# jibo27/3DGS_Hierarchical_Training

Measured on AMD Instinct MI355X. Metric: train-step images/sec + fwd+bwd ms @1M Gaussians, 980x545; 1/2/4/8 GPU, higher is better.
Workload: dtype f32

## Files before the change

3dgs_hierarchical_training_amd/csrc/gsr_kernels.hip:

```cpp
#include <hip/hip_runtime.h>
#include <hip/hip_ext.h>
#include <type_traits>
#include <stdint.h>
#include <stdio.h>
#include <string.h>

#include <algorithm>
#include <atomic>
#include <chrono>
#include <cmath>
#include <map>
#include <mutex>
#include <tuple>
#include <vector>

#include "../../include/gsr.h"
#include "gsr_math.h"
#include "adam_math.h"
#include "radix_sort.h"
#include "blend_common.h"

#ifndef GSR_K9_UNROLL
#define GSR_K9_UNROLL 2
#endif
// ... 1877 lines not shown
    float C0 = 0.f, C1 = 0.f, C2 = 0.f, Dd = 0.f, Aa = 0.f;
    uint32_t last = 0;
    float g0 = 0.f, g1 = 0.f, g2 = 0.f;
    uint32_t lastp = 0u, id_rec = 0u;
    bool uni = false;
    if constexpr (IMP) {
        if (inside) {
            const size_t Pl = (size_t)W * H, P = Pl * (size_t)(T / Tl), pl = (size_t)py * W + px, pid = (size_t)bimg * Pl + pl;
            const float* oc = imp.color + (size_t)bimg * 3 * Pl + pl;
            const float o0 = oc[0], o1 = oc[Pl], o2 = oc[2 * Pl];
            g0 = (o0 >= 0.f && o0 <= 1.f) ? 1.f : 0.f;
            g1 = (o1 >= 0.f && o1 <= 1.f) ? 1.f : 0.f;
            g2 = (o2 >= 0.f && o2 <= 1.f) ? 1.f : 0.f;
            lastp = reinterpret_cast<const uint32_t*>(img)[P + pid];
        }
        const bool want = lastp > 0u && (g0 + g1 + g2) > 0.f;
        if (!__any(want)) return;
        Tr = want ? 1.f : -1.f;
        if (!want) g0 = g1 = g2 = 0.f;
        uni = __all(g0 == g1 && g1 == g2);
        imp.s_sum[0][lane] = 0.f; imp.s_sum[1][lane] = 0.f; imp.s_sum[2][lane] = 0.f;
    }
    float4 ra = {0, 0, 0, 0}, rb = ra, rc = ra;
    constexpr float kL2E = 1.4426950408889634f;
    const float sbx0 = (float)(tx * kTile + (sub & 1) * 8) - 0.5f * (float)W, sby0 = (float)(ty * kTile + (sub >> 1) * 8) - 0.5f * (float)H;
    const float sbx1 = fminf(sbx0 + 7.f, (float)(W - 1) - 0.5f * (float)W), sby1 = fminf(sby0 + 7.f, (float)(H - 1) - 0.5f * (float)H);
    uint32_t id_nn = 0u;
    auto fetch = [&](uint32_t id) {
        const float4* sp = reinterpret_cast<const float4*>(splat + id);
        ra = sp[0]; rb = sp[1]; rc = sp[2];
    };
    if (n > 0) {
        id_rec = list[rg.x + min(lane, n - 1)];
        fetch(id_rec);
        id_nn = list[rg.x + min(NT + lane, n - 1)];
    }
    int batches = 0;
    for (int b = 0; b < nb; b++) {
        const int buf = b & (kFwdBufs - 1);
        if (__all(Tr < 0.f)) break;
        if constexpr (!LEAN) {
        if (ckpt && !(b & 1) && (b >> 1) >= kCkptFirst) {
            float* c = ckpt + ((size_t)(rg.x >> 7) + tile + (b >> 1) - kCkptFirst) * kCkptFloats + sub * 64 + lane;
            c[0] = fabsf(Tr); c[256] = C0; c[512] = C1; c[768] = C2; c[1024] = Dd; c[1280] = Aa;
        }
        }
#ifdef GSR_K6_TIMING
        dbg_mark = __builtin_readcyclecounter();
#endif
        const int cnt = min(NT, n - b * NT);
        const bool reach_me = box_accept(make_tile_test(ra.x, ra.y, ra.z, ra.w, rb.x, rb.y), sbx0, sby0, sbx1, sby1);
        {
            const uint32_t lo = __float_as_uint(rc.w);
            ra.x = pixel_rel(ra.x, pixel_lo_x(lo), tox); ra.y = pixel_rel(ra.y, pixel_lo_y(lo), toy);
        }
        ra.z *= -0.5f * kL2E; ra.w *= -kL2E; rb.x *= -0.5f * kL2E;
        s_ab[buf][lane] = ra; s_ab[kFwdBufs + buf][lane] = rb;
        if constexpr (IMP) imp.s_id[lane] = id_rec;
        else s_c[buf][lane] = make_float2(rc.x, rc.y);
        const unsigned long long reach = __ballot(reach_me && lane < cnt);
        visits += (uint32_t)__popcll(reach);
        __builtin_amdgcn_fence(__ATOMIC_RELEASE, "wavefront");
        __builtin_amdgcn_wave_barrier();
        __builtin_amdgcn_fence(__ATOMIC_ACQUIRE, "wavefront");
        batches = b + 1;
#ifdef GSR_K6_TIMING
        { const unsigned long long t = __builtin_readcyclecounter(); dbg_stage += t - dbg_mark; dbg_mark = t; }
#endif
        const int nxt = (b + 1) * NT + lane;
        fetch(id_nn);
        if constexpr (IMP) id_rec = id_nn;
        id_nn = list[rg.x + min(nxt + NT, n - 1)];
        auto alpha_of = [&](int j, float& p2) {
            const float4 A = s_ab[buf][j];
            const float2 Bq = *reinterpret_cast<const float2*>(&s_ab[kFwdBufs + buf][j]);
            const float dx = A.x - pxf, dy = A.y - pyf;
            p2 = fmaf(Bq.x * dy, dy, fmaf(A.w, dy, A.z * dx) * dx);
#if defined(__HIP_DEVICE_COMPILE__)
            return fminf(kAlphaMax, Bq.y * __builtin_amdgcn_exp2f(p2));
#else
            return fminf(kAlphaMax, Bq.y * exp2f(p2));
#endif
        };
        auto blend = [&](int j, float p2, float alpha) {
            const bool inl = !IMP || (uint32_t)(b * NT + j + 1) <= lastp;
            const bool hit = !(p2 > 0.f) && !(alpha < kAlphaMin) && inl;
#ifdef GSR_K6_TIMING
            dbg_visits++;
#endif
            if constexpr (IMP) {
                if ((__builtin_amdgcn_ballot_w64(!(p2 > 0.f)) & __builtin_amdgcn_ballot_w64(!(alpha < kAlphaMin)) & __builtin_amdgcn_ballot_w64(inl)) == 0ull) return;
            } else {
                if ((__builtin_amdgcn_ballot_w64(!(p2 > 0.f)) & __builtin_amdgcn_ballot_w64(!(alpha < kAlphaMin))) == 0ull) return;
            }
#ifdef GSR_K6_TIMING
            dbg_taken++;
#endif
            const float4 B = s_ab[kFwdBufs + buf][j];
            float2 C = {0.f, 0.f};
            if constexpr (!IMP) C = s_c[buf][j];
            const float am = hit ? alpha : 0.f;
            const float test_T = Tr * (1.f - am);
            const bool pass = !(test_T < kTStop);
            const float asel = pass ? am : 0.f;
            const float w = asel * Tr;
            C0 = fmaf(B.w, w, C0); C1 = fmaf(C.x, w, C1); C2 = fmaf(C.y, w, C2);
            if constexpr (HAS_DA) { Dd = fmaf(B.z, w, Dd); Aa = fmaf(Tr, asel, Aa); }
            Tr = pass ? test_T : -fabsf(Tr);
            last = (pass && hit) ? (uint32_t)(b * NT + j + 1) : last;
            if constexpr (IMP) {
                if (uni) {
                    const float t = wave_reduce_one(w * g0);
                    if (lane == 0) atomicAdd(&imp.s_sum[0][j], t);
                } else {
                    const float t = wave_reduce_three(w * g0, w * g1, w * g2, lane);
                    if (lane < 12 && !(lane & 3)) atomicAdd(&imp.s_sum[lane >> 2][j], t);
                }
            }
        };
        for (unsigned long long rm = reach; rm != 0ull;) {
            const int j = (int)__builtin_ctzll(rm);
#if defined(__HIP_DEVICE_COMPILE__)
            asm("s_bitset0_b64 %0, %1" : "+s"(rm) : "s"(j));
#else
            rm &= rm - 1ull;
#endif
            float p2;
            const float a1 = alpha_of(j, p2);
            blend(j, p2, a1);
        }
#ifdef GSR_K6_TIMING
        dbg_loop += __builtin_readcyclecounter() - dbg_mark;
#endif
        if constexpr (IMP) {
            __builtin_amdgcn_fence(__ATOMIC_RELEASE, "wavefront");
            __builtin_amdgcn_wave_barrier();
            __builtin_amdgcn_fence(__ATOMIC_ACQUIRE, "wavefront");
            const int c = lane & 3;
#pragma unroll
            for (int q = 0; q < 4; q++) {
                const int jj = q * 16 + (lane >> 2);
                if (c < 3 && jj < cnt) {
                    const float v = imp.s_sum[uni ? 0 : c][jj];
                    if (v != 0.f) atomicAdd(imp.S + (size_t)imp.s_id[jj] * kImpStride + c, v);
                }
            }
            __builtin_amdgcn_fence(__ATOMIC_RELEASE, "wavefront");
            __builtin_amdgcn_wave_barrier();
            __builtin_amdgcn_fence(__ATOMIC_ACQUIRE, "wavefront");
            imp.s_sum[0][lane] = 0.f; imp.s_sum[1][lane] = 0.f; imp.s_sum[2][lane] = 0.f;
        }
    }
    if constexpr (IMP) return;
    if constexpr (!LEAN) { if (lane == 0) staged4[tile * 4 + sub] = (uint32_t)min(n, batches * NT); }
    if (cost_out && lane == 0) cost_out[xcd + 8 * kslot] = (uint16_t)min(visits, 65535u);
    if (cut_pass) {
        const bool live = !__all(Tr < 0.f);
        if (lane == 0) {
            if (cut_pass == 1 && live && cut.tend[tile] < cut.tbase[tile + 1]) {
                if (atomicExch(&cut.flag[tile], 1u) == 0u) atomicAdd(&cut.ctl[2], 1u);
            } else {
                uint32_t k = live ? kCutOpenKey : 0u;
                if (!live && batches > 0) {
                    const int lb = batches - 1, lc = min(NT, n - lb * NT);
                    k = __float_as_uint(s_ab[kFwdBufs + (lb & (kFwdBufs - 1))][lc - 1].z);
                }
                const uint32_t e = cut.cur[0] < (uint32_t)kVcEntries ? cut.cur[0] : 0u;
                if (k) atomicMax(cut.key + (size_t)e * (size_t)T + tile, k);
            }
        }
    }
#ifdef GSR_K6_TIMING
    if (lane == 0 && xcd + 8 * kslot < 65536) {
        unsigned long long* d = g_k6_dbg + 4 * (size_t)(xcd + 8 * kslot);
        d[0] = dbg_t0; d[1] = wall_clock64();
        d[2] = ((unsigned long long)__builtin_amdgcn_s_getreg((31 << 11) | 20) << 32) | (unsigned long long)__builtin_amdgcn_s_getreg((31 << 11) | 4);
        d[3] = ((unsigned long long)(uint32_t)n << 32) | (uint32_t)(batches * NT);
        g_k6_cnt[2 * (size_t)(xcd + 8 * kslot)] = dbg_visits; g_k6_cnt[2 * (size_t)(xcd + 8 * kslot) + 1] = dbg_taken;
        g_k6_cyc[2 * (size_t)(xcd + 8 * kslot)] = dbg_stage; g_k6_cyc[2 * (size_t)(xcd + 8 * kslot) + 1] = dbg_loop;
    }
#endif
    if (inside) {
        const size_t Pl = (size_t)W * H, P = Pl * (size_t)(T / Tl), pl = (size_t)py * W + px, pid = (size_t)bimg * Pl + pl;
        const float Tf = fabsf(Tr);
        if constexpr (!LEAN) {
            img[pid] = Tf;
            reinterpret_cast<uint32_t*>(img)[P + pid] = last;
            img[2 * P + pid] = C0; img[3 * P + pid] = C1; img[4 * P + pid] = C2;
            img[5 * P + pid] = Dd; img[6 * P + pid] = Aa;
        }
        float* oc = out_color + (size_t)bimg * 3 * Pl + pl;
        const float o0 = C0 + Tf * bg[0], o1 = C1 + Tf * bg[1], o2 = C2 + Tf * bg[2];
        oc[0] = o0;
        oc[Pl] = o1;
        oc[2 * Pl] = o2;
        if (out_clamped) {
            float* cc = out_clamped + (size_t)bimg * 3 * Pl + pl;
            cc[0] = o0 < 0.f ? 0.f : (o0 > 1.f ? 1.f : o0);
            cc[Pl] = o1 < 0.f ? 0.f : (o1 > 1.f ? 1.f : o1);
            cc[2 * Pl] = o2 < 0.f ? 0.f : (o2 > 1.f ? 1.f : o2);
        }
        if constexpr (HAS_DA) {
            out_depth[pid] = Dd;
            out_alpha[pid] = Aa;
        }
    }
}


__device__ __forceinline__ void blend_fwd_slot(const BlendBalance& bb, const bool table, int& kslot, uint16_t*& cost_out)
{
    if (bb.hdr) {
// ... 1548 lines not shown

#ifdef GSR_K8_PHASES
int gsr_debug_k8_phases(unsigned long long* host_dst) { return (int)hipMemcpyFromSymbol(host_dst, HIP_SYMBOL(g_k8ph), sizeof(unsigned long long) * 8 * 8192); }
#endif
#ifdef GSR_OS_TIMING
int gsr_debug_os_timing(unsigned long long* host_dst) { return (int)hipMemcpyFromSymbol(host_dst, HIP_SYMBOL(g_os_dbg), sizeof(unsigned long long) * 8 * 4096); }
int gsr_debug_gh_timing(unsigned long long* host_dst) { return (int)hipMemcpyFromSymbol(host_dst, HIP_SYMBOL(g_gh_dbg), sizeof(unsigned long long) * 8 * 512); }
#endif
#ifdef GSR_K9_TIMING
int gsr_debug_k9_timing(unsigned long long* host_dst, int reset)
{
    (void)reset;
    return (int)hipMemcpyFromSymbol(host_dst, HIP_SYMBOL(g_k9_dbg), sizeof(unsigned long long) * 8 * kK9DbgWaves);
}
#endif
#ifdef GSR_DB_TIMING
int gsr_debug_db_timing(unsigned long long* host_dst) { return (int)hipMemcpyFromSymbol(host_dst, HIP_SYMBOL(g_db_dbg), sizeof(unsigned long long) * 16); }
#endif
#ifdef GSR_K6_TIMING
int gsr_debug_k6_timing(unsigned long long* host_dst, int blocks)
{
    return (int)hipMemcpyFromSymbol(host_dst, HIP_SYMBOL(g_k6_dbg), sizeof(unsigned long long) * 4 * (size_t)blocks);
}
int gsr_debug_k6_counts(uint32_t* host_dst, int blocks)
{
    return (int)hipMemcpyFromSymbol(host_dst, HIP_SYMBOL(g_k6_cnt), sizeof(uint32_t) * 2 * (size_t)blocks);
}
int gsr_debug_k6_cycles(unsigned long long* host_dst, int blocks)
{
    return (int)hipMemcpyFromSymbol(host_dst, HIP_SYMBOL(g_k6_cyc), sizeof(unsigned long long) * 2 * (size_t)blocks);
}
int gsr_debug_k8_timing(unsigned long long* host_dst, int blocks)
{
    return (int)hipMemcpyFromSymbol(host_dst, HIP_SYMBOL(g_k8_dbg), sizeof(unsigned long long) * 4 * (size_t)blocks);
}
#endif
int gsr_set_option(const char* name, int value)
{
    if (!name) return GSR_ERR_ARG;
    if (!strcmp(name, "blend_fwd_ppt")) return (value == 0 || value == 7) ? GSR_OK : GSR_ERR_ARG;
    if (!strcmp(name, "ab_variants")) return 0;
    if (!strcmp(name, "bwd_split")) { if (value < 0 || value > 64) return GSR_ERR_ARG; g_bwd_split = value; return GSR_OK; }
    if (!strcmp(name, "ckpt_first")) { if (value < 1 || value > 64) return GSR_ERR_ARG; g_ckpt_first = value; return GSR_OK; }
    if (!strcmp(name, "tile_map")) return value == 2 ? GSR_OK : GSR_ERR_ARG;
    if (!strcmp(name, "blend_balance")) { g_blend_balance = value ? 1 : 0; return GSR_OK; }
    if (!strcmp(name, "early_r")) { g_early_r = value ? 1 : 0; return GSR_OK; }
    if (!strcmp(name, "list_cut")) { g_list_cut = value < 0 || value > 2 ? 1 : value; return GSR_OK; }
    if (!strcmp(name, "list_cut_min_n")) { g_list_cut_min_n = value < 0 ? 2000000 : value; return GSR_OK; }
    if (!strcmp(name, "view_cache_reset")) {
        int dev_id = 0;
        if (hipGetDevice(&dev_id) != hipSuccess || hipDeviceSynchronize() != hipSuccess) return GSR_ERR_HIP;
        std::lock_guard<std::mutex> lk(g_state_mutex);
        for (auto& c : g_view_costs)
            if (c.dev == dev_id && hipMemset(c.mem, 0, c.bytes) != hipSuccess) return GSR_ERR_HIP;
        return GSR_OK;
    }
    if (!strcmp(name, "list_cut_margin_e3")) { g_list_cut_margin_e3 = value < 0 ? 50 : value; return GSR_OK; }
    if (!strcmp(name, "list_cut_deep")) { g_list_cut_deep = value < 0 ? 8 : value; return GSR_OK; }
    if (!strcmp(name, "debug_late_bias")) { g_debug_late_bias = value; return GSR_OK; }
    if (!strcmp(name, "tile_sort")) { if (value < 0 || value > 2) return GSR_ERR_ARG; g_tile_sort = value; return GSR_OK; }
    if (!strcmp(name, "tile_sort_max_avg")) { if (value < 0) return GSR_ERR_ARG; g_tile_sort_max_avg = value; return GSR_OK; }
    if (!strcmp(name, "view_pose_tol_e6")) { if (value < 0) return GSR_ERR_ARG; g_view_pose_tol_e6 = value; return GSR_OK; }
    if (!strcmp(name, "depth_sort9")) { g_depth_sort9 = value ? 1 : 0; return GSR_OK; }
    if (!strcmp(name, "direct_binning")) { g_direct_bin = value ? 1 : 0; return GSR_OK; }
    if (!strcmp(name, "speculative_binning")) { g_speculate = value ? 1 : 0; return GSR_OK; }
    if (!strcmp(name, "deterministic_backward")) { g_deterministic = value ? 1 : 0; return GSR_OK; }
    if (!strcmp(name, "binning_capacity_hint")) {
        std::lock_guard<std::mutex> lk(g_state_mutex);
        g_hint_override = value > 0 ? value : -1;
        return GSR_OK;
    }
    if (!strcmp(name, "reset_speculation")) {
        std::lock_guard<std::mutex> lk(g_state_mutex);
        g_hints.clear(); g_hint_override = -1;
        g_spec_overflows = 0; g_spec_forwards = 0; g_exact_forwards = 0; g_depth_window_resorts = 0;
        g_full_depth_sort.clear();
        return GSR_OK;
    }
    if (!strcmp(name, "profile")) { g_profile = (value == 2 || value == 3) ? value : (value ? 1 : 0); g_profile_tick = 0; return GSR_OK; }
    if (!strcmp(name, "prep_hist_max_n")) { g_prep_hist_max_n = value; return GSR_OK; }
    if (!strcmp(name, "small_sort9")) { if (value < 0) return GSR_ERR_ARG; g_small_sort9 = value; return GSR_OK; }
    if (!strcmp(name, "poll_iters")) { g_poll_iters = value < 0 ? 0 : value; return GSR_OK; }
    if (!strcmp(name, "emit_hist")) { g_emit_hist = value ? 1 : 0; return GSR_OK; }
    if (!strcmp(name, "sort_algo")) return value == 2 ? GSR_OK : GSR_ERR_ARG;
    if (!strcmp(name, "blend_bwd_ppt")) return (value == 0 || value == 2) ? GSR_OK : GSR_ERR_ARG;
    return GSR_ERR_ARG;
}

struct DirectBinScratch { size_t M, GT, tbase, bsum, cut_chunk, cut_tend, cut_flag, cut_ctl, cut_bkey, cut_hist, bytes; };
static bool direct_bin_geometry(int N, int T, DirectBin& db, DirectBinScratch& ds)
{
    if (N < 1 || T < 1 || T > kDbMaxTiles) return false;
    static std::atomic<int> cus_cached{0};
    int cus = cus_cached.load(std::memory_order_relaxed);
    if (!cus) {
        int dev = 0, n = 0;
        cus = (hipGetDevice(&dev) == hipSuccess && hipDeviceGetAttribute(&n, hipDeviceAttributeMultiprocessorCount, dev) == hipSuccess && n > 0) ? n : 256;
        cus_cached.store(cus, std::memory_order_relaxed);
    }
    db.N = N; db.T = T; db.Tp = (T + 63) & ~63;
    const int lds = 12 * db.Tp + 4 * kDbPairs;
    const int per_cu = std::min(16, (160 * 1024) / lds);
    const long long resident = std::max<long long>(1, (long long)cus * per_cu);
    const int min_s = 128;
    long long S = ((long long)N + resident - 1) / resident;
    S = std::max<long long>(min_s, (S + 63) & ~63ll);
    if (S > 65472) return false;
    db.S = (int)S;
    db.NC = (int)(((long long)N + S - 1) / S);
    int G = 1;
    while (G * G < db.NC) G++;
    db.Cg = std::max(1, std::min((db.NC + G - 1) / G, 65535 / db.S));
    db.G = (db.NC + db.Cg - 1) / db.Cg;
    if (db.G > kDbMaxGroups) return false;
    size_t o = 0;
    ds.M = o; o += align256((size_t)db.NC * db.Tp * sizeof(uint16_t));
    ds.GT = o; o += align256((size_t)db.G * db.Tp * sizeof(uint32_t));
    ds.tbase = o; o += align256((size_t)(db.Tp + 1) * sizeof(uint32_t));
    ds.bsum = o; o += align256((size_t)db.G * ((db.Tp + 255) / 256) * sizeof(uint32_t));
    ds.cut_chunk = o; o += align256((size_t)db.Tp * sizeof(uint16_t));
    ds.cut_tend = o; o += align256((size_t)db.Tp * sizeof(uint32_t));
    ds.cut_flag = o; o += align256((size_t)db.Tp * sizeof(uint32_t));
    ds.cut_ctl = o; o += 256;
    ds.cut_bkey = o; o += align256((size_t)db.NC * sizeof(uint32_t));
    ds.cut_hist = o; o += align256((size_t)db.NC * sizeof(uint32_t));
    ds.bytes = o;
    return true;
}

static int forward_impl(const GsrForwardArgs* a, const int32_t* retired_at, int64_t retire_step, GsrForwardOut* out, void* stream_)
{
    CallTimer call_timer(g_fwd_calls, g_fwd_ns);
    hipStream_t st = (hipStream_t)stream_;
    if (!a || !out) return fail(GSR_ERR_ARG, "null args%s");
    int rc = check_common(a->N, a->M, a->D, a->W, a->H);
    if (rc) return rc;
    const bool ro = a->render_only != 0;
    if (retired_at) {
        if (ro) return fail(GSR_ERR_ARG, "retired_at: a retire table is not served with render_only (no training step, nothing to retire)%s");
        if (retire_step < 1 || retire_step > 0x7fffffffll) return fail(GSR_ERR_ARG, "retired_at: retire_step must be the 1-based step of the call%s");
    }
    if (ro) {
        if ((a->out_depth == nullptr) != (a->out_alpha == nullptr))
            return fail(GSR_ERR_ARG, "render_only: out_depth and out_alpha are given both or neither%s");
        if ((a->batch && a->batch->B > 1) || a->prepared)
            return fail(GSR_ERR_ARG, "render_only is not served with a batch of B > 1 or a prepared buffer%s");
        if (!a->out_color || !a->bg || !a->alloc) return fail(GSR_ERR_ARG, "missing output / workspace pointer%s");
    } else if (!a->out_color || !a->out_depth || !a->out_alpha || !a->image || !a->bg || !a->alloc)
        return fail(GSR_ERR_ARG, "missing output / workspace pointer%s");
    const int N = a->N, W = a->W, H = a->H;
    BatchDev bt;
    rc = batch_dev(a->batch, N, H, bt);
    if (rc) return rc;
    const int NB = bt.B;
    const int opt_ckpt = g_ckpt_first;
    const int tiles_x = (W + kTile - 1) / kTile, tiles_y = (H + kTile - 1) / kTile, T = tiles_x * tiles_y * NB;
    if (a->sh_origin && (!a->shs || NB > 1 || a->prepared))
        return fail(GSR_ERR_ARG, "sh_origin needs shs and is not served with a batch of B > 1 or a prepared buffer%s");
    out->num_rendered = 0; out->binning = nullptr; out->binning_bytes = 0; out->binning_capacity = 0;
    out->forward_flags = pack_fwd_flags(opt_ckpt) | (ro ? GSR_FWD_FLAG_RENDER_ONLY : 0);
    uint64_t R = 0;
    BlendBalance bb = {};
    ListCut lc = {};
    uint64_t lc_capacity = 0;
    Splat* splat = static_cast<Splat*>(a->geom);
    float* img = static_cast<float*>(a->image);
// ... 934 lines not shown
```

3dgs_hierarchical_training_amd/csrc/radix_sort.h:

```cpp
#pragma once
#include <map>
#include <mutex>
#include <utility>
#include <hip/hip_runtime.h>
#include <stdint.h>

namespace gsr {

__device__ __forceinline__ unsigned long long lanemask_lt()
{
    const unsigned lane = __builtin_amdgcn_mbcnt_hi(~0u, __builtin_amdgcn_mbcnt_lo(~0u, 0u));
    return (1ull << lane) - 1ull;
}

template <int IPT, int NB>
__device__ __forceinline__ void wave_rank(unsigned long long* s_mask, uint32_t* s_cnt, const uint32_t (&dig)[IPT],
                                          uint32_t (&rnk)[IPT], int lane)
{
#pragma unroll
    for (int k = 0; k < NB / 64; k++) { s_mask[k * 64 + lane] = 0ull; s_cnt[k * 64 + lane] = 0u; }
    __builtin_amdgcn_wave_barrier();
    const unsigned long long bit = 1ull << lane, lt = bit - 1ull;
    volatile unsigned long long* vmask = s_mask;
    volatile uint32_t* vcnt = s_cnt;
#pragma unroll
    for (int r = 0; r < IPT; r++) {
        const uint32_t d = dig[r];
        uint32_t below, group;
        const uint32_t base = vcnt[d];
        if (__all(d == (uint32_t)__builtin_amdgcn_readfirstlane((int)d))) {
            below = (uint32_t)lane; group = 64u;
        } else {
            const unsigned long long before = vmask[d];
            atomicXor(&s_mask[d], bit);
            const unsigned long long peers = before ^ vmask[d];
            below = (uint32_t)__popcll(peers & lt);
            group = (uint32_t)__popcll(peers);
        }
        rnk[r] = base + below;
        __builtin_amdgcn_wave_barrier();
        if (below == 0u) vcnt[d] = base + group;
        __builtin_amdgcn_wave_barrier();
    }
}

template <int WAVES>
__device__ __forceinline__ uint32_t block_scan_excl(uint32_t v, uint32_t* s_wsum , int tid)
{
    const int lane = tid & 63, wave = tid >> 6;
    uint32_t inc = v;
#pragma unroll
    for (int off = 1; off < 64; off <<= 1) {
        const uint32_t t = (uint32_t)__shfl_up((int)inc, off, 64);
        if (lane >= off) inc += t;
    }
    if (lane == 63) s_wsum[wave] = inc;
    __syncthreads();
    uint32_t add = 0;
#pragma unroll
    for (int w = 0; w < WAVES; w++) add += (w < wave) ? s_wsum[w] : 0u;
    __syncthreads();
    return add + inc - v;
}

template <typename KeyT> struct OsCfg { static constexpr int kThreads = 512, kTile = 5120; };
template <> struct OsCfg<uint32_t> { static constexpr int kThreads = 1024, kTile = 4096; };

template <typename KernelT>
inline uint32_t onesweep_resident_blocks(KernelT kernel, int threads)
{
    static std::mutex mu;
    static std::map<std::pair<int, const void*>, uint32_t> cache;
    int dev = 0;
    if (hipGetDevice(&dev) != hipSuccess) return 0;
    const auto key = std::make_pair(dev, reinterpret_cast<const void*>(kernel));
    std::lock_guard<std::mutex> lk(mu);
    auto it = cache.find(key);
    if (it != cache.end()) return it->second;
    int per_cu = 0, cus = 0;
    uint32_t v = 0;
    if (hipOccupancyMaxActiveBlocksPerMultiprocessor(&per_cu, kernel, threads, 0) == hipSuccess &&
        hipDeviceGetAttribute(&cus, hipDeviceAttributeMultiprocessorCount, dev) == hipSuccess && per_cu > 0 && cus > 0)
        v = (uint32_t)per_cu * (uint32_t)cus;
    cache[key] = v;
    return v;
}
__device__ unsigned int g_onesweep_giveups = 0u;
struct OsRider;
constexpr int kOsRanges = 32;
constexpr uint32_t kOsLocal = 1u << 30, kOsIncl = 2u << 30, kOsMask = (1u << 30) - 1u;
constexpr uint32_t kOsTicketWords = (4 * kOsRanges + 63) / 64 * 64;
constexpr uint32_t kOnesweepHeadWords = 4 * kOsRanges * 256 + kOsTicketWords;
constexpr uint32_t kOnesweepHeadWords9 = 3 * kOsRanges * 512 + kOsTicketWords;
constexpr uint32_t kOnesweepHeadWordsMax = kOnesweepHeadWords9 > kOnesweepHeadWords ? kOnesweepHeadWords9 : kOnesweepHeadWords;
inline unsigned int* onesweep_overflow_word(void* scratch) { return static_cast<unsigned int*>(scratch) + 3 * kOsRanges * 512 + 100; }

template <typename KeyT>
__host__ __device__ inline uint32_t onesweep_run_len(uint32_t n)
{
    constexpr uint64_t kT = (uint64_t)OsCfg<KeyT>::kTile;
    const uint64_t ntiles = ((uint64_t)n + kT - 1) / kT, per = (ntiles + kOsRanges - 1) / kOsRanges;
    return (uint32_t)(per * kT);
}
__host__ __device__ inline int onesweep_passes(int bits) { return (bits + 7) / 8; }
__host__ __device__ inline int onesweep_dbits(int bits) { const int p = onesweep_passes(bits); return (bits + p - 1) / p; }
template <typename KeyT>
__host__ __device__ inline uint32_t onesweep_status_words(uint32_t capacity, int bits)
{
    const uint32_t nblocks = (capacity + OsCfg<KeyT>::kTile - 1) / OsCfg<KeyT>::kTile;
    return (uint32_t)((size_t)onesweep_passes(bits) * nblocks * 256);
}
__host__ __device__ inline uint32_t* onesweep_status(void* scratch) { return static_cast<uint32_t*>(scratch) + kOnesweepHeadWords; }

struct OsRider {
    const uint2* parts;
    uint32_t nparts;
    unsigned long long* host;
    unsigned long long seq;
};
__device__ __forceinline__ void onesweep_rider_publish(const OsRider& rd, unsigned long long (*s_r)[16]);

#ifdef GSR_OS_TIMING
__device__ unsigned long long g_gh_dbg[512 * 8];
#endif
template <typename KeyT, int PASSES, int GS = 256>
__global__ __launch_bounds__(256) void k_radix_ghist(const KeyT* __restrict__ keys, uint32_t n, int begin_bit,
                                                     uint32_t* __restrict__ ghist ,
                                                     const unsigned long long* __restrict__ n_dev,
                                                     uint32_t* __restrict__ status, uint32_t status_words, int dbits, int bits, uint32_t bias = 0u,
                                                     uint32_t kclamp = 0xffffffffu, unsigned int* __restrict__ overflow = nullptr, OsRider rider = OsRider{})
{
#ifdef GSR_OS_TIMING
    unsigned long long ght[8] = {0, 0, 0, 0, 0, 0, 0, 0}, ght_last = __builtin_readcyclecounter();
    ght[6] = ght_last;
#define GH_T(k) do { const unsigned long long now_ = __builtin_readcyclecounter(); ght[k] += now_ - ght_last; ght_last = now_; } while (0)
#else
#define GH_T(k) do { } while (0)
#endif
    if (rider.host && blockIdx.x == gridDim.x - 1) {
        __shared__ unsigned long long s_r[2][16];
        onesweep_rider_publish(rider, s_r);
    }
    GH_T(0);
    uint32_t dmask[PASSES];
#pragma unroll
    for (int p = 0; p < PASSES; p++) dmask[p] = (1u << min(dbits, bits - dbits * p)) - 1u;
    if (n_dev) n = (uint32_t)min((unsigned long long)n, *n_dev);
    for (uint32_t q = blockIdx.x * 256 + threadIdx.x; q < status_words / 4; q += gridDim.x * 256)
        reinterpret_cast<uint4*>(status)[q] = make_uint4(0u, 0u, 0u, 0u);
    __shared__ uint32_t h[PASSES][GS];
    const int tid = threadIdx.x;
    bool beyond = false;
#pragma unroll
    for (int p = 0; p < PASSES; p++)
        for (int d = tid; d < GS; d += 256) h[p][d] = 0;
    __syncthreads();
    GH_T(1);
    constexpr uint64_t kT = (uint64_t)OsCfg<KeyT>::kTile;
    const uint64_t ntiles = ((uint64_t)n + kT - 1) / kT, per = (ntiles + kOsRanges - 1) / kOsRanges;
    const uint32_t bpr = gridDim.x / kOsRanges, x = blockIdx.x / bpr, sub = blockIdx.x - x * bpr;
    const uint64_t lo = min((uint64_t)n, (uint64_t)x * per * kT), hi = min((uint64_t)n, (uint64_t)(x + 1) * per * kT);
    constexpr int KPV = 16 / (int)sizeof(KeyT);
    const KeyT* kr = keys + lo;
    const uint32_t len = (uint32_t)(hi - lo);
    const uint32_t nv = (((uintptr_t)kr & 15) == 0) ? len / KPV : 0u;
    const uint4* k4 = reinterpret_cast<const uint4*>(kr);
    for (uint32_t i0 = sub * 256 + tid; i0 < nv; i0 += 4u * bpr * 256u) {
        uint4 qq[4];
#pragma unroll
        for (int u = 0; u < 4; u++) {
            const uint32_t i = i0 + (uint32_t)u * bpr * 256u;
            qq[u] = k4[i < nv ? i : i0];
        }
#pragma unroll
        for (int u = 0; u < 4; u++) {
            if (i0 + (uint32_t)u * bpr * 256u >= nv) break;
            const uint32_t w[4] = {qq[u].x, qq[u].y, qq[u].z, qq[u].w};
#pragma unroll
            for (int c = 0; c < 4; c++) {
#pragma unroll
                for (int e = 0; e < KPV / 4; e++) {
                    const uint32_t kraw = (uint32_t)(sizeof(KeyT) == 4 ? w[c] : ((w[c] >> (16 * e)) & 0xffffu));
                    beyond |= (kraw - bias > kclamp) && kraw != (uint32_t)(KeyT)~(KeyT)0;
                    const uint32_t k = min(kraw - bias, kclamp) >> begin_bit;
#pragma unroll
                    for (int p = 0; p < PASSES; p++) atomicAdd(&h[p][(k >> (dbits * p)) & dmask[p]], 1u);
                }
            }
        }
    }
    for (uint32_t i = nv * KPV + sub * 256 + tid; i < len; i += bpr * 256) {
        const uint32_t kraw = (uint32_t)kr[i];
        beyond |= (kraw - bias > kclamp) && kraw != (uint32_t)(KeyT)~(KeyT)0;
        const uint32_t k = min(kraw - bias, kclamp) >> begin_bit;
#pragma unroll
        for (int p = 0; p < PASSES; p++) atomicAdd(&h[p][(k >> (dbits * p)) & dmask[p]], 1u);
    }
    if (overflow && __any(beyond) && (threadIdx.x & 63) == 0) atomicAdd(overflow, 1u);
    GH_T(2);
    __syncthreads();
    GH_T(3);
#pragma unroll
    for (int p = 0; p < PASSES; p++)
        for (int d = tid; d < GS; d += 256)
            if (h[p][d]) atomicAdd(&ghist[(p * kOsRanges + x) * GS + d], h[p][d]);
#ifdef GSR_OS_TIMING
    GH_T(4);
    asm volatile("s_waitcnt vmcnt(0)" ::: "memory");
    GH_T(5);
    if (tid == 0 && blockIdx.x < 512) { ght[7] = ght_last; for (int q = 0; q < 8; q++) g_gh_dbg[blockIdx.x * 8 + q] = ght[q]; }
#endif
}

__device__ __forceinline__ void onesweep_rider_publish(const OsRider& rd, unsigned long long (*s_r)[16])
{
    unsigned long long a = 0ull, b = 0ull;
    for (uint32_t q0 = threadIdx.x; q0 < rd.nparts; q0 += 8u * blockDim.x) {
        uint2 v[8];
#pragma unroll
        for (int u = 0; u < 8; u++) {
            const uint32_t q = q0 + (uint32_t)u * blockDim.x;
            v[u] = q < rd.nparts ? rd.parts[q] : make_uint2(0u, 0u);
        }
#pragma unroll
        for (int u = 0; u < 8; u++) { a += v[u].x; b += v[u].y; }
    }
#pragma unroll
    for (int off = 32; off > 0; off >>= 1) { a += __shfl_xor(a, off, 64); b += __shfl_xor(b, off, 64); }
    if ((threadIdx.x & 63u) == 0u) { s_r[0][threadIdx.x >> 6] = a; s_r[1][threadIdx.x >> 6] = b; }
    __syncthreads();
    if (threadIdx.x == 0) {
        a = b = 0ull;
        for (uint32_t w = 0; w < blockDim.x / 64u; w++) { a += s_r[0][w]; b += s_r[1][w]; }
        __atomic_store_n(rd.host + 2, (unsigned long long)g_onesweep_giveups, __ATOMIC_RELAXED);
        __atomic_store_n(rd.host + 3, b, __ATOMIC_RELAXED);
        __atomic_store_n(rd.host, a, __ATOMIC_RELAXED);
        __threadfence_system();
        __atomic_store_n(rd.host + 1, rd.seq, __ATOMIC_RELAXED);
        __threadfence_system();
    }
}

constexpr int kOsTile = 4096;

#ifdef GSR_OS_TIMING
__device__ unsigned long long g_os_dbg[4096 * 8];
#define OS_T(k) do { const unsigned long long now_ = __builtin_readcyclecounter(); if (threadIdx.x == 0) ost[k] += now_ - ost_last; ost_last = now_; } while (0)
#else
#define OS_T(k) do { } while (0)
#endif
template <typename KeyT, int NB>
__global__ __launch_bounds__(OsCfg<KeyT>::kThreads) void k_onesweep(const KeyT* __restrict__ kin, const uint32_t* __restrict__ vin,
                                                         KeyT* __restrict__ kout, uint32_t* __restrict__ vout, uint32_t n, int shift,
                                                         const uint32_t* __restrict__ ghist ,
                                                         uint32_t* __restrict__ status ,
                                                         uint32_t* __restrict__ ticket,
                                                         const unsigned long long* __restrict__ n_dev, uint32_t dmask, int runs,
                                                         uint32_t bias = 0u, uint32_t kclamp = 0xffffffffu, OsRider rider = OsRider{})
{
    constexpr int GS = NB > 256 ? NB : 256;
    constexpr int kOsThreads = OsCfg<KeyT>::kThreads, kOsTile = OsCfg<KeyT>::kTile, kOsIPT = kOsTile / kOsThreads, kOsWaves = kOsThreads / 64;
    if (rider.host && blockIdx.x == gridDim.x - 1) {
        __shared__ unsigned long long s_r[2][16];
        onesweep_rider_publish(rider, s_r);
    }
    if (n_dev) n = (uint32_t)min((unsigned long long)n, *n_dev);
    __shared__ unsigned long long s_mask[kOsWaves][NB];
    __shared__ uint32_t s_cnt[kOsWaves][NB];
    __shared__ KeyT s_keys[kOsTile];
    __shared__ uint32_t s_vals[kOsTile];
    __shared__ uint32_t s_start[NB];
    __shared__ uint32_t s_gbase[NB];
    __shared__ uint32_t s_wsum[kOsWaves];
    __shared__ uint32_t s_tile;
    const int tid = threadIdx.x, wave = tid >> 6, lane = tid & 63;
#ifdef GSR_OS_TIMING
    unsigned long long ost[8] = {0, 0, 0, 0, 0, 0, 0, 0}, ost_last = __builtin_readcyclecounter();
    ost[6] = ost_last;
#endif
    const uint32_t ntiles = (uint32_t)(((uint64_t)n + kOsTile - 1) / kOsTile);
    const uint32_t per = runs > 1 ? (ntiles + kOsRanges - 1) / kOsRanges : ntiles;
    const uint32_t run = runs > 1 ? (blockIdx.x & (kOsRanges - 1)) : 0u;
    uint32_t krun = runs > 1 ? blockIdx.x / kOsRanges : blockIdx.x;
    if (ticket) {
        if (tid == 0) s_tile = atomicAdd(ticket + run, 1u);
        __syncthreads();
        krun = s_tile;
    }
    const uint32_t run_start = run * per;
    const uint32_t tile = run_start + krun;
    if (krun >= per || tile >= ntiles) return;
    const uint32_t base = tile * (uint32_t)kOsTile;
    const uint32_t valid = min((uint32_t)kOsTile, n - base);
    KeyT key[kOsIPT];
    uint32_t val[kOsIPT], dig[kOsIPT], rnk[kOsIPT];
#pragma unroll
    for (int r = 0; r < kOsIPT; r++) {
        const uint32_t p = (uint32_t)(wave * (kOsIPT * 64) + r * 64 + lane);
        if (p < valid) {
            key[r] = kin[base + p];
            val[r] = vin[base + p];
            dig[r] = (min((uint32_t)key[r] - bias, kclamp) >> shift) & dmask;
        } else {
            key[r] = (KeyT)~(KeyT)0; val[r] = 0u; dig[r] = (uint32_t)(NB - 1);
        }
    }
    OS_T(0);
    wave_rank<kOsIPT, NB>(s_mask[wave], s_cnt[wave], dig, rnk, lane);
    __syncthreads();
    OS_T(1);
    const bool is_digit = tid < NB;
    uint32_t mine = 0;
    if (is_digit) {
#pragma unroll
        for (int w = 0; w < kOsWaves; w++) {
            const uint32_t c = s_cnt[w][tid];
            s_cnt[w][tid] = mine;
            mine += c;
        }
    }
    const uint32_t real = (tid == NB - 1) ? mine - ((uint32_t)kOsTile - valid) : mine;
    uint32_t* my_status = status + (size_t)tile * GS + (tid & (NB - 1));
    if (is_digit) __hip_atomic_store(my_status, kOsLocal | real, __ATOMIC_RELAXED, __HIP_MEMORY_SCOPE_AGENT);
    const uint32_t lstart = block_scan_excl<kOsWaves>(mine, s_wsum, tid);
    uint32_t gtot = 0u, gpre = 0u;
    if (is_digit) {
#pragma unroll
        for (int x = 0; x < kOsRanges; x++) {
            const uint32_t c = ghist[x * GS + tid];
            gtot += c;
            gpre += (uint32_t)x < run ? c : 0u;
        }
    }
    const uint32_t dbase = block_scan_excl<kOsWaves>(gtot, s_wsum, tid) + gpre;
    OS_T(2);
    if (is_digit) {
        uint32_t excl = 0, polls = 0;
        const int t_lo = (int)run_start;
        for (int t = (int)tile - 1; t >= t_lo;) {
            constexpr int kWin = 4;
            uint32_t v[kWin];
#pragma unroll
            for (int q = 0; q < kWin; q++)
                v[q] = (t - q >= t_lo) ? __hip_atomic_load(status + (size_t)(t - q) * GS + tid, __ATOMIC_RELAXED, __HIP_MEMORY_SCOPE_AGENT) : kOsIncl;
            bool done = false;
#pragma unroll
            for (int q = 0; q < kWin; q++) {
                if (done) break;
                const uint32_t f = v[q] & ~kOsMask;
                if (f == 0u) { done = true; break; }
                excl += v[q] & kOsMask;
                t--;
                if (f == kOsIncl) { t = t_lo - 1; done = true; }
            }
            if (t >= t_lo && done) {
                __builtin_amdgcn_s_sleep(1);
                if (++polls > (1u << 23)) { atomicAdd(&g_onesweep_giveups, 1u); break; }
            }
        }
        __hip_atomic_store(my_status, kOsIncl | (excl + real), __ATOMIC_RELAXED, __HIP_MEMORY_SCOPE_AGENT);
        s_start[tid] = lstart;
        s_gbase[tid] = dbase + excl - lstart;
    }
    __syncthreads();
    OS_T(3);
#pragma unroll
    for (int r = 0; r < kOsIPT; r++) {
        const uint32_t lp = s_start[dig[r]] + s_cnt[wave][dig[r]] + rnk[r];
        s_keys[lp] = key[r];
        s_vals[lp] = val[r];
    }
    __syncthreads();
    OS_T(4);
#pragma unroll
    for (int r = 0; r < kOsIPT; r++) {
        const uint32_t p = r * kOsThreads + tid;
        if (p < valid) {
            const KeyT k = s_keys[p];
            const uint32_t d = (min((uint32_t)k - bias, kclamp) >> shift) & dmask;
            const uint32_t g = s_gbase[d] + p;
            kout[g] = k;
            vout[g] = s_vals[p];
        }
    }
#ifdef GSR_OS_TIMING
    OS_T(5);
    if (tid == 0 && sizeof(KeyT) == 4 && blockIdx.x < 4096) { ost[7] = ost_last; for (int q = 0; q < 8; q++) g_os_dbg[blockIdx.x * 8 + q] = ost[q]; }
#endif
}

inline size_t onesweep_scratch_bytes(uint32_t n)
{
    const size_t nblocks = ((size_t)n + kOsTile - 1) / kOsTile;
    const size_t nb = nblocks ? nblocks : 1;
    const size_t w8 = kOnesweepHeadWords + 4 * nb * 256, w9 = kOnesweepHeadWords9 + 3 * nb * 512;
    return ((w8 > w9 ? w8 : w9) * sizeof(uint32_t) + 255) & ~(size_t)255;
}

template <typename KeyT>
inline hipError_t onesweep_sort_pairs(KeyT* keys, uint32_t* vals, KeyT* keys_alt, uint32_t* vals_alt, uint32_t n, int begin_bit,
                                      int end_bit, void* scratch, int* in_alt, hipStream_t stream,
                                      const unsigned long long* n_dev = nullptr, bool head_prezeroed = false, bool hist_done = false,
                                      int max_digit_bits = 8, uint32_t bias = 0u, const OsRider* rider = nullptr)
{
    const bool wide = max_digit_bits == 9;
    const OsRider rd = (rider && (wide || !hist_done)) ? *rider : OsRider{};
    const OsRider rd0 = (rider && !wide && hist_done) ? *rider : OsRider{};
    *in_alt = 0;
    if (n == 0) return hipSuccess;
    const int bits = end_bit - begin_bit;
    const int passes = (bits + (wide ? 9 : 8) - 1) / (wide ? 9 : 8);
    if (passes < 1 || passes > 4 || (wide && (passes != 3 || sizeof(KeyT) != 4 || hist_done || begin_bit != 0))) return hipErrorInvalidValue;
    const uint32_t GS = wide ? 512u : 256u;
    const uint32_t kclamp = (wide && bits < 32) ? ((1u << bits) - 1u) : 0xffffffffu;
    if (!wide) bias = 0u;
    const int dbits = (bits + passes - 1) / passes;
    const uint32_t nblocks = (n + OsCfg<KeyT>::kTile - 1) / OsCfg<KeyT>::kTile;
    uint32_t* ghist = static_cast<uint32_t*>(scratch);
    uint32_t* tickets = ghist + (wide ? 3 * kOsRanges * 512 : 4 * kOsRanges * 256);
    uint32_t* status = tickets + kOsTicketWords;
    if (!head_prezeroed && !hist_done) {
        hipError_t e = hipMemsetAsync(scratch, 0, (wide ? kOnesweepHeadWords9 : kOnesweepHeadWords) * sizeof(uint32_t), stream);
        if (e != hipSuccess) return e;
    }
    const uint32_t status_words = (uint32_t)((size_t)passes * nblocks * GS);
    const uint32_t per_cap = (nblocks + kOsRanges - 1) / kOsRanges;
    const uint32_t hgrid = kOsRanges * (per_cap < 32u ? per_cap : 32u);
    if (wide)
        hipLaunchKernelGGL((k_radix_ghist<KeyT, 3, 512>), dim3(hgrid), dim3(256), 0, stream, keys, n, begin_bit, ghist, n_dev, status, status_words, dbits, bits,
                           bias, kclamp, onesweep_overflow_word(scratch), rd);
    else if (!hist_done)
    switch (passes) {
        case 1: hipLaunchKernelGGL((k_radix_ghist<KeyT, 1>), dim3(hgrid), dim3(256), 0, stream, keys, n, begin_bit, ghist, n_dev, status, status_words, dbits, bits, 0u, 0xffffffffu, (unsigned int*)nullptr, rd); break;
        case 2: hipLaunchKernelGGL((k_radix_ghist<KeyT, 2>), dim3(hgrid), dim3(256), 0, stream, keys, n, begin_bit, ghist, n_dev, status, status_words, dbits, bits, 0u, 0xffffffffu, (unsigned int*)nullptr, rd); break;
        case 3: hipLaunchKernelGGL((k_radix_ghist<KeyT, 3>), dim3(hgrid), dim3(256), 0, stream, keys, n, begin_bit, ghist, n_dev, status, status_words, dbits, bits, 0u, 0xffffffffu, (unsigned int*)nullptr, rd); break;
        default: hipLaunchKernelGGL((k_radix_ghist<KeyT, 4>), dim3(hgrid), dim3(256), 0, stream, keys, n, begin_bit, ghist, n_dev, status, status_words, dbits, bits, 0u, 0xffffffffu, (unsigned int*)nullptr, rd); break;
    }
    KeyT *kin = keys, *kout = keys_alt;
    uint32_t *vin = vals, *vout = vals_alt;
    for (int p = 0; p < passes; p++) {
        const uint32_t pmask = (1u << (dbits < bits - dbits * p ? dbits : bits - dbits * p)) - 1u;
        const int runs = p == 0 ? kOsRanges : 1;
        const uint32_t pgrid = runs > 1 ? kOsRanges * per_cap : nblocks;
        const int wbits = dbits < bits - dbits * p ? dbits : bits - dbits * p;
        const uint32_t resident = wbits <= 6 ? onesweep_resident_blocks(k_onesweep<KeyT, 64>, OsCfg<KeyT>::kThreads)
                                             : onesweep_resident_blocks(k_onesweep<KeyT, 256>, OsCfg<KeyT>::kThreads);
        uint32_t* tk_p = pgrid <= resident ? (uint32_t*)nullptr : tickets + p * kOsRanges;
        if (wide) {
            const uint32_t res9 = onesweep_resident_blocks(k_onesweep<KeyT, 512>, OsCfg<KeyT>::kThreads);
            uint32_t* tk9 = pgrid <= res9 ? (uint32_t*)nullptr : tickets + p * kOsRanges;
            hipLaunchKernelGGL((k_onesweep<KeyT, 512>), dim3(pgrid), dim3(OsCfg<KeyT>::kThreads), 0, stream, kin, vin, kout, vout, n,
                               begin_bit + dbits * p, ghist + p * kOsRanges * 512, status + (size_t)p * nblocks * 512, tk9, n_dev, pmask, runs, bias, kclamp);
        } else if (wbits <= 6)
            hipLaunchKernelGGL((k_onesweep<KeyT, 64>), dim3(pgrid), dim3(OsCfg<KeyT>::kThreads), 0, stream, kin, vin, kout, vout, n,
                               begin_bit + dbits * p, ghist + p * kOsRanges * 256, status + (size_t)p * nblocks * 256, tk_p, n_dev, pmask, runs,
                               0u, 0xffffffffu, p == 0 ? rd0 : OsRider{});
        else
            hipLaunchKernelGGL((k_onesweep<KeyT, 256>), dim3(pgrid), dim3(OsCfg<KeyT>::kThreads), 0, stream, kin, vin, kout, vout, n,
                               begin_bit + dbits * p, ghist + p * kOsRanges * 256, status + (size_t)p * nblocks * 256, tk_p, n_dev, pmask, runs,
                               0u, 0xffffffffu, p == 0 ? rd0 : OsRider{});
        KeyT* tk = kin; kin = kout; kout = tk;
        uint32_t* tv = vin; vin = vout; vout = tv;
        *in_alt ^= 1;
    }
    return hipGetLastError();
}

}
```

Baseline: 1282.

## Add grouped decoupled-lookback to onesweep sort, early-exit blend, dedicated rider block

```diff
diff --git a/3dgs_hierarchical_training_amd/csrc/gsr_kernels.hip b/3dgs_hierarchical_training_amd/csrc/gsr_kernels.hip
--- a/3dgs_hierarchical_training_amd/csrc/gsr_kernels.hip
+++ b/3dgs_hierarchical_training_amd/csrc/gsr_kernels.hip
@@ -1983,7 +1983,7 @@
             return fminf(kAlphaMax, Bq.y * exp2f(p2));
 #endif
         };
-        auto blend = [&](int j, float p2, float alpha) {
+        auto blend = [&](int j, float p2, float alpha, unsigned long long& rm) {
             const bool inl = !IMP || (uint32_t)(b * NT + j + 1) <= lastp;
             const bool hit = !(p2 > 0.f) && !(alpha < kAlphaMin) && inl;
 #ifdef GSR_K6_TIMING
@@ -2018,6 +2018,11 @@
                     if (lane < 12 && !(lane & 3)) atomicAdd(&imp.s_sum[lane >> 2][j], t);
                 }
             }
+#if defined(__HIP_DEVICE_COMPILE__)
+            asm("s_cmp_lg_u64 %1, 0\n\ts_cselect_b64 %0, %0, 0" : "+s"(rm) : "s"(__builtin_amdgcn_ballot_w64(pass)) : "scc");
+#else
+            rm = __builtin_amdgcn_ballot_w64(pass) == 0ull ? 0ull : rm;
+#endif
         };
         for (unsigned long long rm = reach; rm != 0ull;) {
             const int j = (int)__builtin_ctzll(rm);
@@ -2028,7 +2033,7 @@
 #endif
             float p2;
             const float a1 = alpha_of(j, p2);
-            blend(j, p2, a1);
+            blend(j, p2, a1, rm);
         }
 #ifdef GSR_K6_TIMING
         dbg_loop += __builtin_readcyclecounter() - dbg_mark;
@@ -3743,6 +3748,12 @@
     if (!strcmp(name, "small_sort9")) { if (value < 0) return GSR_ERR_ARG; g_small_sort9 = value; return GSR_OK; }
     if (!strcmp(name, "poll_iters")) { g_poll_iters = value < 0 ? 0 : value; return GSR_OK; }
     if (!strcmp(name, "emit_hist")) { g_emit_hist = value ? 1 : 0; return GSR_OK; }
+    if (!strcmp(name, "sort_group")) {
+        if (value < 0 || value > 64 || (value & (value - 1)) || value == 1) return GSR_ERR_ARG;
+        g_os_force_group = value;
+        return GSR_OK;
+    }
+    if (!strcmp(name, "sort_tickets")) { g_os_force_tickets = value ? 1 : 0; return GSR_OK; }
     if (!strcmp(name, "sort_algo")) return value == 2 ? GSR_OK : GSR_ERR_ARG;
     if (!strcmp(name, "blend_bwd_ppt")) return (value == 0 || value == 2) ? GSR_OK : GSR_ERR_ARG;
     return GSR_ERR_ARG;
diff --git a/3dgs_hierarchical_training_amd/csrc/radix_sort.h b/3dgs_hierarchical_training_amd/csrc/radix_sort.h
--- a/3dgs_hierarchical_training_amd/csrc/radix_sort.h
+++ b/3dgs_hierarchical_training_amd/csrc/radix_sort.h
@@ -88,7 +88,16 @@
 __device__ unsigned int g_onesweep_giveups = 0u;
 struct OsRider;
 constexpr int kOsRanges = 32;
-constexpr uint32_t kOsLocal = 1u << 30, kOsIncl = 2u << 30, kOsMask = (1u << 30) - 1u;
+constexpr uint32_t kOsLocal = 1u << 30, kOsIncl = 2u << 30, kOsAgg = kOsLocal | kOsIncl, kOsMask = (1u << 30) - 1u;
+inline int g_os_force_group = 0;
+inline int g_os_force_tickets = 0;
+inline int onesweep_group(uint32_t chain)
+{
+    if (g_os_force_group > 0) return g_os_force_group;
+    int g = 4;
+    while (g < 64 && 2u * (uint32_t)g * (uint32_t)g < chain) g <<= 1;
+    return g;
+}
 constexpr uint32_t kOsTicketWords = (4 * kOsRanges + 63) / 64 * 64;
 constexpr uint32_t kOnesweepHeadWords = 4 * kOsRanges * 256 + kOsTicketWords;
 constexpr uint32_t kOnesweepHeadWords9 = 3 * kOsRanges * 512 + kOsTicketWords;
@@ -118,6 +127,7 @@
     unsigned long long* host;
     unsigned long long seq;
 };
+template <bool WIDE = false>
 __device__ __forceinline__ void onesweep_rider_publish(const OsRider& rd, unsigned long long (*s_r)[16]);
 
 #ifdef GSR_OS_TIMING
@@ -137,16 +147,18 @@
 #else
 #define GH_T(k) do { } while (0)
 #endif
-    if (rider.host && blockIdx.x == gridDim.x - 1) {
+    const uint32_t hgrid = gridDim.x - (rider.host ? 1u : 0u);
+    if (blockIdx.x == hgrid) {
         __shared__ unsigned long long s_r[2][16];
-        onesweep_rider_publish(rider, s_r);
+        onesweep_rider_publish<true>(rider, s_r);
+        return;
     }
     GH_T(0);
     uint32_t dmask[PASSES];
 #pragma unroll
     for (int p = 0; p < PASSES; p++) dmask[p] = (1u << min(dbits, bits - dbits * p)) - 1u;
     if (n_dev) n = (uint32_t)min((unsigned long long)n, *n_dev);
-    for (uint32_t q = blockIdx.x * 256 + threadIdx.x; q < status_words / 4; q += gridDim.x * 256)
+    for (uint32_t q = blockIdx.x * 256 + threadIdx.x; q < status_words / 4; q += hgrid * 256)
         reinterpret_cast<uint4*>(status)[q] = make_uint4(0u, 0u, 0u, 0u);
     __shared__ uint32_t h[PASSES][GS];
     const int tid = threadIdx.x;
@@ -158,7 +170,7 @@
     GH_T(1);
     constexpr uint64_t kT = (uint64_t)OsCfg<KeyT>::kTile;
     const uint64_t ntiles = ((uint64_t)n + kT - 1) / kT, per = (ntiles + kOsRanges - 1) / kOsRanges;
-    const uint32_t bpr = gridDim.x / kOsRanges, x = blockIdx.x / bpr, sub = blockIdx.x - x * bpr;
+    const uint32_t bpr = hgrid / kOsRanges, x = blockIdx.x / bpr, sub = blockIdx.x - x * bpr;
     const uint64_t lo = min((uint64_t)n, (uint64_t)x * per * kT), hi = min((uint64_t)n, (uint64_t)(x + 1) * per * kT);
     constexpr int KPV = 16 / (int)sizeof(KeyT);
     const KeyT* kr = keys + lo;
@@ -212,9 +224,25 @@
 #endif
 }
 
+template <bool WIDE>
 __device__ __forceinline__ void onesweep_rider_publish(const OsRider& rd, unsigned long long (*s_r)[16])
 {
     unsigned long long a = 0ull, b = 0ull;
+    if constexpr (WIDE) {
+        const uint32_t npairs = (((uintptr_t)rd.parts & 15) == 0) ? rd.nparts / 2u : 0u;
+        const uint4* p4 = reinterpret_cast<const uint4*>(rd.parts);
+        for (uint32_t q0 = threadIdx.x; q0 < npairs; q0 += 16u * blockDim.x) {
+            uint4 v[16];
+#pragma unroll
+            for (int u = 0; u < 16; u++) {
+                const uint32_t q = q0 + (uint32_t)u * blockDim.x;
+                v[u] = q < npairs ? p4[q] : make_uint4(0u, 0u, 0u, 0u);
+            }
+#pragma unroll
+            for (int u = 0; u < 16; u++) { a += v[u].x; a += v[u].z; b += v[u].y; b += v[u].w; }
+        }
+        for (uint32_t q = 2u * npairs + threadIdx.x; q < rd.nparts; q += blockDim.x) { const uint2 v = rd.parts[q]; a += v.x; b += v.y; }
+    } else {
     for (uint32_t q0 = threadIdx.x; q0 < rd.nparts; q0 += 8u * blockDim.x) {
         uint2 v[8];
 #pragma unroll
@@ -224,6 +252,7 @@
         }
 #pragma unroll
         for (int u = 0; u < 8; u++) { a += v[u].x; b += v[u].y; }
+    }
     }
 #pragma unroll
     for (int off = 32; off > 0; off >>= 1) { a += __shfl_xor(a, off, 64); b += __shfl_xor(b, off, 64); }
@@ -255,7 +284,7 @@
                                                          const uint32_t* __restrict__ ghist ,
                                                          uint32_t* __restrict__ status ,
                                                          uint32_t* __restrict__ ticket,
-                                                         const unsigned long long* __restrict__ n_dev, uint32_t dmask, int runs,
+                                                         const unsigned long long* __restrict__ n_dev, uint32_t dmask, int runs, int group,
                                                          uint32_t bias = 0u, uint32_t kclamp = 0xffffffffu, OsRider rider = OsRider{})
 {
     constexpr int GS = NB > 256 ? NB : 256;
@@ -305,11 +334,16 @@
             key[r] = (KeyT)~(KeyT)0; val[r] = 0u; dig[r] = (uint32_t)(NB - 1);
         }
     }
+    const bool is_digit = __builtin_amdgcn_readfirstlane(wave) < NB / 64;
+    uint32_t gh[kOsRanges];
+    if (is_digit) {
+#pragma unroll
+        for (int x = 0; x < kOsRanges; x++) gh[x] = ghist[x * GS + tid];
+    }
     OS_T(0);
     wave_rank<kOsIPT, NB>(s_mask[wave], s_cnt[wave], dig, rnk, lane);
     __syncthreads();
     OS_T(1);
-    const bool is_digit = tid < NB;
     uint32_t mine = 0;
     if (is_digit) {
 #pragma unroll
@@ -327,7 +361,7 @@
     if (is_digit) {
 #pragma unroll
         for (int x = 0; x < kOsRanges; x++) {
-            const uint32_t c = ghist[x * GS + tid];
+            const uint32_t c = gh[x];
             gtot += c;
             gpre += (uint32_t)x < run ? c : 0u;
         }
@@ -337,25 +371,55 @@
     if (is_digit) {
         uint32_t excl = 0, polls = 0;
         const int t_lo = (int)run_start;
-        for (int t = (int)tile - 1; t >= t_lo;) {
-            constexpr int kWin = 4;
+        const uint32_t chain = min(per, ntiles - run_start);
+        const bool grouped = chain > 2u * (uint32_t)group;
+        const int g_lo = grouped ? t_lo + (int)(krun / (uint32_t)group) * group : t_lo;
+        const bool g_last = grouped && (krun % (uint32_t)group) == (uint32_t)group - 1u;
+        bool closed = g_lo == t_lo, gaveup = false;
+        for (int t = (int)tile - 1; t >= g_lo;) {
+            constexpr int kWin = 8;
             uint32_t v[kWin];
 #pragma unroll
             for (int q = 0; q < kWin; q++)
-                v[q] = (t - q >= t_lo) ? __hip_atomic_load(status + (size_t)(t - q) * GS + tid, __ATOMIC_RELAXED, __HIP_MEMORY_SCOPE_AGENT) : kOsIncl;
+                v[q] = (t - q >= g_lo) ? __hip_atomic_load(status + (size_t)(t - q) * GS + tid, __ATOMIC_RELAXED, __HIP_MEMORY_SCOPE_AGENT) : kOsIncl;
             bool done = false;
 #pragma unroll
             for (int q = 0; q < kWin; q++) {
                 if (done) break;
                 const uint32_t f = v[q] & ~kOsMask;
                 if (f == 0u) { done = true; break; }
+                const bool word = t >= g_lo;
                 excl += v[q] & kOsMask;
                 t--;
-                if (f == kOsIncl) { t = t_lo - 1; done = true; }
+                if (f == kOsIncl) { closed = closed || word; t = g_lo - 1; done = true; }
             }
-            if (t >= t_lo && done) {
+            if (t >= g_lo && done) {
                 __builtin_amdgcn_s_sleep(1);
-                if (++polls > (1u << 23)) { atomicAdd(&g_onesweep_giveups, 1u); break; }
+                if (++polls > (1u << 23)) { atomicAdd(&g_onesweep_giveups, 1u); gaveup = true; break; }
+            }
+        }
+        if (!closed && !gaveup) {
+            if (g_last) __hip_atomic_store(my_status, kOsAgg | (excl + real), __ATOMIC_RELAXED, __HIP_MEMORY_SCOPE_AGENT);
+            for (int u = g_lo - 1; u >= t_lo;) {
+                constexpr int kWin = 8;
+                uint32_t v[kWin];
+#pragma unroll
+                for (int q = 0; q < kWin; q++)
+                    v[q] = (u - q * group >= t_lo) ? __hip_atomic_load(status + (size_t)(u - q * group) * GS + tid, __ATOMIC_RELAXED, __HIP_MEMORY_SCOPE_AGENT) : kOsIncl;
+                bool done = false;
+#pragma unroll
+                for (int q = 0; q < kWin; q++) {
+                    if (done) break;
+                    const uint32_t f = v[q] & ~kOsMask;
+                    if (f == 0u || f == kOsLocal) { done = true; break; }
+                    excl += v[q] & kOsMask;
+                    u -= group;
+                    if (f == kOsIncl) { u = t_lo - 1; done = true; }
+                }
+                if (u >= t_lo && done) {
+                    __builtin_amdgcn_s_sleep(1);
+                    if (++polls > (1u << 23)) { atomicAdd(&g_onesweep_giveups, 1u); break; }
+                }
             }
         }
         __hip_atomic_store(my_status, kOsIncl | (excl + real), __ATOMIC_RELAXED, __HIP_MEMORY_SCOPE_AGENT);
@@ -427,14 +491,14 @@
     const uint32_t per_cap = (nblocks + kOsRanges - 1) / kOsRanges;
     const uint32_t hgrid = kOsRanges * (per_cap < 32u ? per_cap : 32u);
     if (wide)
-        hipLaunchKernelGGL((k_radix_ghist<KeyT, 3, 512>), dim3(hgrid), dim3(256), 0, stream, keys, n, begin_bit, ghist, n_dev, status, status_words, dbits, bits,
+        hipLaunchKernelGGL((k_radix_ghist<KeyT, 3, 512>), dim3(hgrid + (rd.host ? 1u : 0u)), dim3(256), 0, stream, keys, n, begin_bit, ghist, n_dev, status, status_words, dbits, bits,
                            bias, kclamp, onesweep_overflow_word(scratch), rd);
     else if (!hist_done)
     switch (passes) {
-        case 1: hipLaunchKernelGGL((k_radix_ghist<KeyT, 1>), dim3(hgrid), dim3(256), 0, stream, keys, n, begin_bit, ghist, n_dev, status, status_words, dbits, bits, 0u, 0xffffffffu, (unsigned int*)nullptr, rd); break;
-        case 2: hipLaunchKernelGGL((k_radix_ghist<KeyT, 2>), dim3(hgrid), dim3(256), 0, stream, keys, n, begin_bit, ghist, n_dev, status, status_words, dbits, bits, 0u, 0xffffffffu, (unsigned int*)nullptr, rd); break;
-        case 3: hipLaunchKernelGGL((k_radix_ghist<KeyT, 3>), dim3(hgrid), dim3(256), 0, stream, keys, n, begin_bit, ghist, n_dev, status, status_words, dbits, bits, 0u, 0xffffffffu, (unsigned int*)nullptr, rd); break;
-        default: hipLaunchKernelGGL((k_radix_ghist<KeyT, 4>), dim3(hgrid), dim3(256), 0, stream, keys, n, begin_bit, ghist, n_dev, status, status_words, dbits, bits, 0u, 0xffffffffu, (unsigned int*)nullptr, rd); break;
+        case 1: hipLaunchKernelGGL((k_radix_ghist<KeyT, 1>), dim3(hgrid + (rd.host ? 1u : 0u)), dim3(256), 0, stream, keys, n, begin_bit, ghist, n_dev, status, status_words, dbits, bits, 0u, 0xffffffffu, (unsigned int*)nullptr, rd); break;
+        case 2: hipLaunchKernelGGL((k_radix_ghist<KeyT, 2>), dim3(hgrid + (rd.host ? 1u : 0u)), dim3(256), 0, stream, keys, n, begin_bit, ghist, n_dev, status, status_words, dbits, bits, 0u, 0xffffffffu, (unsigned int*)nullptr, rd); break;
+        case 3: hipLaunchKernelGGL((k_radix_ghist<KeyT, 3>), dim3(hgrid + (rd.host ? 1u : 0u)), dim3(256), 0, stream, keys, n, begin_bit, ghist, n_dev, status, status_words, dbits, bits, 0u, 0xffffffffu, (unsigned int*)nullptr, rd); break;
+        default: hipLaunchKernelGGL((k_radix_ghist<KeyT, 4>), dim3(hgrid + (rd.host ? 1u : 0u)), dim3(256), 0, stream, keys, n, begin_bit, ghist, n_dev, status, status_words, dbits, bits, 0u, 0xffffffffu, (unsigned int*)nullptr, rd); break;
     }
     KeyT *kin = keys, *kout = keys_alt;
     uint32_t *vin = vals, *vout = vals_alt;
@@ -445,19 +509,20 @@
         const int wbits = dbits < bits - dbits * p ? dbits : bits - dbits * p;
         const uint32_t resident = wbits <= 6 ? onesweep_resident_blocks(k_onesweep<KeyT, 64>, OsCfg<KeyT>::kThreads)
                                              : onesweep_resident_blocks(k_onesweep<KeyT, 256>, OsCfg<KeyT>::kThreads);
-        uint32_t* tk_p = pgrid <= resident ? (uint32_t*)nullptr : tickets + p * kOsRanges;
+        uint32_t* tk_p = (pgrid <= resident && !g_os_force_tickets) ? (uint32_t*)nullptr : tickets + p * kOsRanges;
+        const int group = onesweep_group(runs > 1 ? per_cap : nblocks);
         if (wide) {
             const uint32_t res9 = onesweep_resident_blocks(k_onesweep<KeyT, 512>, OsCfg<KeyT>::kThreads);
-            uint32_t* tk9 = pgrid <= res9 ? (uint32_t*)nullptr : tickets + p * kOsRanges;
+            uint32_t* tk9 = (pgrid <= res9 && !g_os_force_tickets) ? (uint32_t*)nullptr : tickets + p * kOsRanges;
             hipLaunchKernelGGL((k_onesweep<KeyT, 512>), dim3(pgrid), dim3(OsCfg<KeyT>::kThreads), 0, stream, kin, vin, kout, vout, n,
-                               begin_bit + dbits * p, ghist + p * kOsRanges * 512, status + (size_t)p * nblocks * 512, tk9, n_dev, pmask, runs, bias, kclamp);
+                               begin_bit + dbits * p, ghist + p * kOsRanges * 512, status + (size_t)p * nblocks * 512, tk9, n_dev, pmask, runs, group, bias, kclamp);
         } else if (wbits <= 6)
             hipLaunchKernelGGL((k_onesweep<KeyT, 64>), dim3(pgrid), dim3(OsCfg<KeyT>::kThreads), 0, stream, kin, vin, kout, vout, n,
-                               begin_bit + dbits * p, ghist + p * kOsRanges * 256, status + (size_t)p * nblocks * 256, tk_p, n_dev, pmask, runs,
+                               begin_bit + dbits * p, ghist + p * kOsRanges * 256, status + (size_t)p * nblocks * 256, tk_p, n_dev, pmask, runs, group,
                                0u, 0xffffffffu, p == 0 ? rd0 : OsRider{});
         else
             hipLaunchKernelGGL((k_onesweep<KeyT, 256>), dim3(pgrid), dim3(OsCfg<KeyT>::kThreads), 0, stream, kin, vin, kout, vout, n,
-                               begin_bit + dbits * p, ghist + p * kOsRanges * 256, status + (size_t)p * nblocks * 256, tk_p, n_dev, pmask, runs,
+                               begin_bit + dbits * p, ghist + p * kOsRanges * 256, status + (size_t)p * nblocks * 256, tk_p, n_dev, pmask, runs, group,
                                0u, 0xffffffffu, p == 0 ? rd0 : OsRider{});
         KeyT* tk = kin; kin = kout; kout = tk;
         uint32_t* tv = vin; vin = vout; vout = tv;
```

Result: faster. 1299 (median of 6 runs) (+1.3%).
